# hbb1/2d-gaussian-splatting

Hardware: NVIDIA H100
Metric: fwd+bwd Msplats/sec at 1M surfels/1080p (higher is better)
Workload: dtype f32

## Files before the change

### 2d-gaussian-splatting_b200/csrc/api.cu

```cuda
#include <cstdarg>
#include <cstdio>
#include <cstring>
#include <cstdlib>
#include <algorithm>

#include "../../include/surfel_rasterizer.h"
#include "common.cuh"
#include "kernels.h"

using namespace surfel;

static thread_local char g_err[512] = "";

void surfel_set_error(const char* fmt, ...) {
    va_list ap;
    va_start(ap, fmt);
    vsnprintf(g_err, sizeof(g_err), fmt, ap);
    va_end(ap);
}

namespace {

struct Variants { int sort_radix; };
Variants& variants() {
    static Variants v = [] {
        auto is = [](const char* name, const char* val) { const char* e = getenv(name); return e && !strcmp(e, val) ? 1 : 0; };
        return Variants{is("SURFEL_SORT", "radix")};
    }();
    return v;
}

struct Frame { int W, H, gx, gy, row0, row1, tiles; };

bool frame_of(const surfel_settings_t* s, Frame& f) {
    if (!s) { surfel_set_error("settings is NULL"); return false; }
    f.W = s->image_width; f.H = s->image_height;
    if (f.W <= 0 || f.H <= 0) { surfel_set_error("bad image size %dx%d", f.W, f.H); return false; }
    f.gx = (f.W + kBlockX - 1) / kBlockX; f.gy = (f.H + kBlockY - 1) / kBlockY;
    f.tiles = f.gx * f.gy;
    f.row0 = s->tile_row_begin; f.row1 = s->tile_row_end;
    if (f.row0 == 0 && f.row1 == 0) f.row1 = f.gy;
    if (f.row0 < 0 || f.row1 > f.gy || f.row0 > f.row1) {
        surfel_set_error("bad tile row band [%d,%d) for %d tile rows", f.row0, f.row1, f.gy);
        return false;
    }
    return true;
}

int tile_key_bits(int tiles) {
    int b = 0;
    unsigned n = (unsigned)tiles;
    while (n) { b++; n >>= 1; }
    return 32 + b;
}

BinningLayout binning_layout(size_t R, int tiles) {
    BinningLayout L;
    size_t r = R > 0 ? R : 1, o = 0;
    L.keys_a = o;    o = align_up(o + r * 8, 256);
    L.keys_b = o;    o = align_up(o + r * 8, 256);
    L.vals_a = o;    o = align_up(o + r * 4, 256);
    L.vals_b = o;    o = align_up(o + r * 4, 256);
    L.ranges = o;    o = align_up(o + (size_t)tiles * 8, 256);
    L.sort_temp = o; o = align_up(o + std::max(radix_sort_temp_bytes(r), bucket_temp_bytes(tiles)), 256);
    L.total = o;
    return L;
}

struct BinView { uint64_t *k_unsorted, *k_sorted; uint32_t *v_unsorted, *v_sorted; uint64_t *k_a, *k_b; uint32_t *v_a, *v_b; uint2* ranges; void* temp; };

BinView bin_view(void* ws, size_t R, const Frame& f) {
    BinningLayout L = binning_layout(R, f.tiles);
    char* c = (char*)ws;
    BinView v;
    v.k_a = (uint64_t*)(c + L.keys_a); v.k_b = (uint64_t*)(c + L.keys_b);
    v.v_a = (uint32_t*)(c + L.vals_a); v.v_b = (uint32_t*)(c + L.vals_b);
    const bool in_b = radix_sort_passes(tile_key_bits(f.tiles)) & 1;
    v.k_unsorted = v.k_a; v.v_unsorted = v.v_a;
    v.k_sorted = in_b ? v.k_b : v.k_a; v.v_sorted = in_b ? v.v_b : v.v_a;
    v.ranges = (uint2*)(c + L.ranges);
    v.temp = c + L.sort_temp;
    return v;
}

uint32_t* mapped_alias(uint32_t* host) {
    if (!host) return nullptr;
    cudaPointerAttributes a;
    if (cudaPointerGetAttributes(&a, host) == cudaSuccess && a.type == cudaMemoryTypeHost && a.devicePointer)
        return (uint32_t*)a.devicePointer;
    (void)cudaGetLastError();
    return nullptr;
}

}

extern "C" {

int surfel_abi_version(void) { return SURFEL_ABI_VERSION; }

int surfel_set_variant(const char* name, const char* value) {
    if (!name || !value) { surfel_set_error("surfel_set_variant: NULL argument"); return 1; }
    Variants& v = variants();
    if (!strcmp(name, "sort")) {
        if (!strcmp(value, "bucket")) v.sort_radix = 0; else if (!strcmp(value, "radix")) v.sort_radix = 1; else goto bad;
    } else goto bad;
    return 0;
bad:
    surfel_set_error("surfel_set_variant: unknown variant %s=%s", name, value);
    return 1;
}
const char* surfel_last_error(void) { return g_err; }

int surfel_accepts_capacity(void) { return variants().sort_radix ? 0 : 1; }

size_t surfel_geom_bytes(int P) { return geom_layout(P).total; }
size_t surfel_image_bytes(int W, int H) { return image_layout(W, H).total; }
size_t surfel_binning_bytes(size_t R, int W, int H) {
    const int tiles = ((W + kBlockX - 1) / kBlockX) * ((H + kBlockY - 1) / kBlockY);
    return binning_layout(R, tiles).total;
}

int surfel_geom_offsets(int P, size_t* out) {
    GeomLayout L = geom_layout(P);
    out[0] = L.rec; out[1] = L.tiles_touched; out[2] = L.offsets; out[3] = L.clamped; out[4] = L.counters;
    out[5] = L.tmat;
    return 0;
}
int surfel_binning_offsets(size_t R, int W, int H, size_t* out) {
    const int tiles = ((W + kBlockX - 1) / kBlockX) * ((H + kBlockY - 1) / kBlockY);
    BinningLayout L = binning_layout(R, tiles);
    const bool in_b = radix_sort_passes(tile_key_bits(tiles)) & 1;
    out[0] = L.keys_a; out[1] = L.vals_a;
    out[2] = in_b ? L.keys_b : L.keys_a; out[3] = in_b ? L.vals_b : L.vals_a;
    out[4] = L.ranges;
    return 0;
}
int surfel_image_offsets(int W, int H, size_t* out) {
    ImageLayout L = image_layout(W, H);
    out[0] = L.accum; out[1] = L.n_contrib;
    return 0;
}

int surfel_forward_preprocess(const surfel_settings_t* s, int P, int M, const float* means3D,
                              const float* opacities, const float* scales, const float* rotations,
                              const float* transMat_precomp, const float* shs,
                              const float* colors_precomp, int32_t* radii, void* geom_ws, void* image_ws,
                              uint32_t* num_rendered_host, void* stream) {
    Frame f;
    if (!frame_of(s, f)) return 1;
    cudaStream_t st = (cudaStream_t)stream;
    if (P < 0) { surfel_set_error("P < 0"); return 1; }
    if (P > 0 && (!means3D || !opacities || !radii || !geom_ws)) { surfel_set_error("NULL required pointer"); return 1; }
    if (P > 0 && !transMat_precomp && (!scales || !rotations)) { surfel_set_error("need scales+rotations or transMat_precomp"); return 1; }
    if (P > 0 && !colors_precomp && !shs) { surfel_set_error("need shs or colors_precomp"); return 1; }
    if (!colors_precomp && (s->sh_degree < 0 || s->sh_degree > 3 || (s->sh_degree + 1) * (s->sh_degree + 1) > M)) {
        surfel_set_error("sh_degree %d unsupported for M=%d coefficients (max degree 3)", s->sh_degree, M);
        return 1;
    }
    GeomLayout L = geom_layout(P);
    char* g = (char*)geom_ws;
    if (P == 0) {
        if (num_rendered_host) *num_rendered_host = 0;
        return 0;
    }
    PreFwdParams p;
    p.P = P; p.D = s->sh_degree; p.M = M; p.W = f.W; p.H = f.H; p.gx = f.gx; p.gy = f.gy;
    p.row0 = f.row0; p.row1 = f.row1; p.prefiltered = s->prefiltered; p.scale_modifier = s->scale_modifier;
    p.means3D = means3D; p.scales = scales; p.rotations = rotations; p.opacities = opacities;
    p.shs = shs; p.transMat_precomp = transMat_precomp; p.colors_precomp = colors_precomp;
    p.viewmatrix = s->viewmatrix; p.projmatrix = s->projmatrix; p.campos = s->campos;
    p.radii = radii; p.rec = (float4*)(g + L.rec); p.tmat = (float4*)(g + L.tmat); p.tiles_touched = (uint32_t*)(g + L.tiles_touched);
    p.offsets = (uint32_t*)(g + L.offsets); p.clamped = (uint8_t*)(g + L.clamped);
    p.scan_status = (unsigned long long*)(g + L.scan_status); p.counters = (uint32_t*)(g + L.counters);
    p.tile_count = image_ws ? (uint32_t*)((char*)image_ws + image_layout(f.W, f.H).tile_count) : nullptr;
    p.num_rendered_mapped = mapped_alias(num_rendered_host);
    if (launch_preprocess_fwd(p, st)) return 1;
    if (num_rendered_host && !p.num_rendered_mapped)
        SURFEL_CUDA_OK(cudaMemcpyAsync(num_rendered_host, p.counters + 1, 4, cudaMemcpyDeviceToHost, st));
    return 0;
}

int surfel_bin_duplicate(const surfel_settings_t* s, int P, uint32_t R, const void* geom_ws,
                         const int32_t* radii, void* binning_ws, void* stream) {
    Frame f;
    if (!frame_of(s, f)) return 1;
    if (R == 0 || P == 0) return 0;
    GeomLayout L = geom_layout(P);
    const char* g = (const char*)geom_ws;
    BinView v = bin_view(binning_ws, R, f);
    return launch_duplicate_with_keys(P, f.gx, f.gy, f.row0, f.row1, (const float4*)(g + L.tmat), radii,
                                      (const uint32_t*)(g + L.offsets), v.k_unsorted, v.v_unsorted,
                                      (cudaStream_t)stream);
}

int surfel_bin_sort(const surfel_settings_t* s, uint32_t R, void* binning_ws, void* stream) {
    Frame f;
    if (!frame_of(s, f)) return 1;
    BinView v = bin_view(binning_ws, R, f);
    if (launch_radix_sort_pairs(v.k_a, v.v_a, v.k_b, v.v_b, R, tile_key_bits(f.tiles), v.temp,
                                (cudaStream_t)stream)) return 1;
    return launch_identify_tile_ranges(R, f.tiles, v.k_sorted, v.ranges, (cudaStream_t)stream);
}

int surfel_render_forward(const surfel_settings_t* s, uint32_t R, const void* geom_ws,
                          const void* binning_ws, void* image_ws, float* out_color,
                          float* out_others, void* stream) {
    Frame f;
    if (!frame_of(s, f)) return 1;
    BinView v = bin_view(const_cast<void*>(binning_ws), R, f);
    ImageLayout I = image_layout(f.W, f.H);
    RenderParams p;
    memset(&p, 0, sizeof(p));
    p.W = f.W; p.H = f.H; p.gx = f.gx; p.gy = f.gy; p.row0 = f.row0; p.row1 = f.row1;
    p.ranges = v.ranges; p.point_list = v.v_sorted;
    p.rec = (const float4*)((const char*)geom_ws + 0);
    p.bg = s->bg;
    p.out_color = out_color; p.out_others = out_others;
    p.out_plane = s->out_plane_stride > 0 ? (size_t)s->out_plane_stride : (size_t)f.W * f.H;
    if (p.out_plane < (size_t)f.W * f.H) { surfel_set_error("out_plane_stride smaller than the image"); return 1; }
    p.rep_count = s->out_replica_count;
    if (p.rep_count < 0 || p.rep_count > SURFEL_MAX_OUT_REPLICAS) { surfel_set_error("out_replica_count out of range"); return 1; }
    if (p.rep_count > 0 && out_others != out_color + 3 * p.out_plane) {
        surfel_set_error("out_replica_base needs out_others == out_color + 3 * out_plane_stride (one 10-plane frame)");
        return 1;
    }
    for (int r = 0; r < SURFEL_MAX_OUT_REPLICAS; r++) {
        p.rep_base[r] = r < p.rep_count ? (unsigned long long)s->out_replica_base[r] : 0ull;
        if (r < p.rep_count && (p.rep_base[r] == 0 || (p.rep_base[r] & 3ull))) { surfel_set_error("out_replica_base: null or misaligned address"); return 1; }
    }
    p.accum = (float*)((char*)image_ws + I.accum); p.n_contrib = (uint32_t*)((char*)image_ws + I.n_contrib);
    return launch_render_fwd(p, (cudaStream_t)stream);
}

int surfel_bin_bucket(const surfel_settings_t* s, int P, uint32_t R, const void* geom_ws,
                      const int32_t* radii, void* binning_ws, const void* image_ws_with_counts,
                      int write_keys, void* stream) {
    Frame f;
    if (!frame_of(s, f)) return 1;
    GeomLayout L = geom_layout(P);
    const char* g = (const char*)geom_ws;
    BinView v = bin_view(binning_ws, R, f);
    unsigned long long* pairs = (unsigned long long*)(v.k_sorted == v.k_a ? v.k_b : v.k_a);
    return launch_bucket_binning(P, R, f.gx, f.gy, f.row0, f.row1, (const float4*)(g + L.tmat), radii,
                                 (const uint32_t*)(g + L.offsets), pairs, v.v_sorted,
                                 write_keys ? (unsigned long long*)v.k_sorted : nullptr, v.ranges, v.temp,
                                 image_ws_with_counts ? (const uint32_t*)((const char*)image_ws_with_counts +
                                                                          image_layout(f.W, f.H).tile_count) : nullptr,
                                 (cudaStream_t)stream);
}

int surfel_forward_render(const surfel_settings_t* s, int P, uint32_t R, const int32_t* radii,
                          const void* geom_ws, void* binning_ws, void* image_ws, int tile_counts_ready,
                          float* out_color, float* out_others, void* stream) {
    const bool use_radix = variants().sort_radix != 0;
    if (!use_radix) {
        if (surfel_bin_bucket(s, P, R, geom_ws, radii, binning_ws, tile_counts_ready ? image_ws : nullptr, 0, stream)) return 1;
        return surfel_render_forward(s, R, geom_ws, binning_ws, image_ws, out_color, out_others, stream);
    }
    if (surfel_bin_duplicate(s, P, R, geom_ws, radii, binning_ws, stream)) return 1;
    if (surfel_bin_sort(s, R, binning_ws, stream)) return 1;
    return surfel_render_forward(s, R, geom_ws, binning_ws, image_ws, out_color, out_others, stream);
}

int surfel_backward(const surfel_settings_t* s, int P, int M, uint32_t R, const float* means3D,
                    const float* scales, const float* rotations, const float* transMat_precomp,
                    const float* shs, int has_colors_precomp, const int32_t* radii,
                    const void* geom_ws, const void* binning_ws, const void* image_ws,
                    const float* dL_dout_color, const float* dL_dout_others, float* grad_scratch,
                    float* dL_dmeans2D, float* dL_dcolors, float* dL_dopacity, float* dL_dmeans3D,
                    float* dL_dtransMat, float* dL_dsh, float* dL_dscales, float* dL_drotations,
                    int lowpass_depth_quirk, void* stream) {
    Frame f;
    if (!frame_of(s, f)) return 1;
    if (P <= 0) return 0;
    cudaStream_t st = (cudaStream_t)stream;
    if (!grad_scratch || !dL_dmeans2D || !dL_dopacity || !dL_dmeans3D) { surfel_set_error("NULL required gradient buffer"); return 1; }
    GeomLayout L = geom_layout(P);
    const char* g = (const char*)geom_ws;
    SURFEL_CUDA_OK(cudaMemsetAsync(grad_scratch, 0, (size_t)P * kGradFloats * 4, st));
    if (R > 0) {
        BinView v = bin_view(const_cast<void*>(binning_ws), R, f);
        ImageLayout I = image_layout(f.W, f.H);
        RenderParams p;
        memset(&p, 0, sizeof(p));
        p.W = f.W; p.H = f.H; p.gx = f.gx; p.gy = f.gy; p.row0 = f.row0; p.row1 = f.row1;
        p.ranges = v.ranges; p.point_list = v.v_sorted; p.rec = (const float4*)(g + L.rec); p.bg = s->bg;
        p.accum = (float*)((char*)image_ws + I.accum); p.n_contrib = (uint32_t*)((char*)image_ws + I.n_contrib);
        p.dL_dpix = dL_dout_color; p.dL_dothers = dL_dout_others; p.grad_rec = grad_scratch;
        p.grad_plane = s->grad_plane_stride > 0 ? (size_t)s->grad_plane_stride : (size_t)f.W * f.H;
        if (p.grad_plane < (size_t)f.W * f.H) { surfel_set_error("grad_plane_stride smaller than the image"); return 1; }
        p.lowpass_quirk = lowpass_depth_quirk;
        if (launch_render_bwd(p, st)) return 1;
    }
    PreBwdParams q;
    memset(&q, 0, sizeof(q));
    q.P = P; q.D = s->sh_degree; q.M = M; q.W = f.W; q.H = f.H; q.scale_modifier = s->scale_modifier;
    q.means3D = means3D; q.scales = scales; q.rotations = rotations; q.shs = shs;
    q.transMat_precomp = transMat_precomp; q.has_colors_precomp = has_colors_precomp;
    q.viewmatrix = s->viewmatrix; q.projmatrix = s->projmatrix; q.campos = s->campos;
    q.radii = radii; q.tmat = (const float4*)(g + L.tmat); q.clamped = (const uint8_t*)(g + L.clamped);
    q.grad_rec = grad_scratch;
    q.dL_dmeans2D = dL_dmeans2D; q.dL_dcolors = dL_dcolors; q.dL_dopacity = dL_dopacity;
    q.dL_dmeans3D = dL_dmeans3D; q.dL_dtransMat = dL_dtransMat; q.dL_dsh = dL_dsh;
    q.dL_dscales = dL_dscales; q.dL_drots = dL_drotations;
    q.defer_sh = (s->sh_grad_deferred && shs != nullptr && !has_colors_precomp) ? 1 : 0;
    if (q.defer_sh && !dL_dcolors) { surfel_set_error("sh_grad_deferred needs dL_dcolors"); return 1; }
    return launch_preprocess_bwd(q, st);
}

int surfel_sh_grad_expand(int P, int M, int sh_degree, const float* means3D, const float* campos,
                          const float* dL_dcolors, float* dL_dsh, void* stream) {
    if (P <= 0 || M <= 0) return 0;
    if (!means3D || !campos || !dL_dcolors || !dL_dsh) { surfel_set_error("surfel_sh_grad_expand: NULL argument"); return 1; }
    if (sh_degree < 0 || sh_degree > 3 || (sh_degree + 1) * (sh_degree + 1) > M) { surfel_set_error("surfel_sh_grad_expand: degree / M mismatch"); return 1; }
    return launch_sh_grad_expand(P, M, sh_degree, means3D, campos, dL_dcolors, dL_dsh, (cudaStream_t)stream);
}

int surfel_mark_visible(int P, const float* means3D, const float* viewmatrix,
                        const float* projmatrix, uint8_t* present, void* stream) {
    (void)projmatrix;
    return launch_mark_visible(P, means3D, viewmatrix, present, (cudaStream_t)stream);
}

size_t surfel_sort_temp_bytes(size_t n) { return radix_sort_temp_bytes(n); }
int surfel_grad_scratch_floats(void) { return kGradFloats; }

int surfel_sort_pairs(uint64_t* keys_a, uint32_t* vals_a, uint64_t* keys_b, uint32_t* vals_b,
                      size_t n, int end_bit, void* temp, int* result_in_b, void* stream) {
    if (result_in_b) *result_in_b = radix_sort_passes(end_bit) & 1;
    return launch_radix_sort_pairs(keys_a, vals_a, keys_b, vals_b, n, end_bit, temp, (cudaStream_t)stream);
}

}
```

### 2d-gaussian-splatting_b200/csrc/common.cuh

```cuda
#pragma once
#include <cuda_runtime.h>
#include <stdint.h>

namespace surfel {

constexpr int kBlockX = 16;
constexpr int kBlockY = 16;
constexpr int kTilePixels = kBlockX * kBlockY;
constexpr float kNear = 0.2f;
constexpr float kFar = 100.0f;
constexpr float kFilterSize = 0.707106f;
constexpr float kFilterInvSquare = 2.0f;
constexpr float kCutoff = 3.0f;
constexpr float kAlphaMax = 0.99f;
constexpr float kAlphaMin = 1.0f / 255.0f;
constexpr float kTMin = 0.0001f;

constexpr int kChDepth = 0, kChAlpha = 1, kChNormal = 2, kChMidDepth = 5, kChDistortion = 6;

constexpr int kRecQuads = 8;
constexpr int kRecBytes = kRecQuads * 16;
constexpr int kRecQuadsFwd = 5;
constexpr int kRecQuadsBwd = 6;

constexpr int kTmQuads = 3;

constexpr int kGradFloats = 24;
constexpr int kGradUsed = 22;

struct GeomLayout {
    size_t rec, tmat, tiles_touched, offsets, clamped, scan_status, counters, total;
};
struct ImageLayout {
    size_t accum, n_contrib, tile_count, total;
};
struct BinningLayout {
    size_t keys_a, keys_b, vals_a, vals_b, ranges, sort_temp, total;
};

__host__ __device__ inline size_t align_up(size_t x, size_t a) { return (x + a - 1) / a * a; }

constexpr int kPreBlock = 128;

inline GeomLayout geom_layout(int P) {
    GeomLayout L;
    size_t o = 0;
    size_t p = (size_t)(P > 0 ? P : 1);
    L.rec = o;            o = align_up(o + p * kRecBytes, 256);
    L.tmat = o;           o = align_up(o + p * kTmQuads * 16, 256);
    L.tiles_touched = o;  o = align_up(o + p * 4, 256);
    L.offsets = o;        o = align_up(o + p * 4, 256);
    L.clamped = o;        o = align_up(o + p, 256);
    L.scan_status = o;    o = align_up(o + ((p + kPreBlock - 1) / kPreBlock + 1) * 8, 256);
    L.counters = o;       o = align_up(o + 64, 256);
    L.total = o;
    return L;
}
inline ImageLayout image_layout(int W, int H) {
    ImageLayout L;
    size_t n = (size_t)W * (size_t)H;
    size_t o = 0;
    L.accum = o;      o = align_up(o + n * 3 * 4, 256);
    L.n_contrib = o;  o = align_up(o + n * 2 * 4, 256);
    const size_t tiles = (size_t)((W + kBlockX - 1) / kBlockX) * (size_t)((H + kBlockY - 1) / kBlockY);
    L.tile_count = o; o = align_up(o + tiles * 4, 256);
    L.total = o;
    return L;
}

__device__ __forceinline__ int f2i_sat(float x) { return __float2int_rz(x); }

__device__ __forceinline__ void get_rect(float cx, float cy, int radius, int gx, int gy, int row0,
                                         int row1, int& x0, int& y0, int& x1, int& y1) {
    const float r = (float)radius;
    x0 = min(gx, max(0, f2i_sat((cx - r) / (float)kBlockX)));
    y0 = min(gy, max(0, f2i_sat((cy - r) / (float)kBlockY)));
    x1 = min(gx, max(0, f2i_sat(((cx + r) + (float)(kBlockX - 1)) / (float)kBlockX)));
    y1 = min(gy, max(0, f2i_sat(((cy + r) + (float)(kBlockY - 1)) / (float)kBlockY)));
    y0 = min(row1, max(row0, y0));
    y1 = min(row1, max(row0, y1));
}

__device__ __forceinline__ float4 ld_nc_f4(const float4* p) {
    float4 r;
    asm volatile("ld.global.nc.L1::no_allocate.v4.f32 {%0,%1,%2,%3}, [%4];"
                 : "=f"(r.x), "=f"(r.y), "=f"(r.z), "=f"(r.w) : "l"(p));
    return r;
}

}

void surfel_set_error(const char* fmt, ...);

constexpr int kMaxDevices = 64;
inline int current_device_slot() {
    int dev = -1;
    if (cudaGetDevice(&dev) != cudaSuccess || dev < 0 || dev >= kMaxDevices) return -1;
    return dev;
}
inline int current_device_sm_count() {
    static int cached[kMaxDevices] = {};
    const int slot = current_device_slot();
    if (slot >= 0 && cached[slot] > 0) return cached[slot];
    int dev = 0, n = 0;
    if (cudaGetDevice(&dev) != cudaSuccess || cudaDeviceGetAttribute(&n, cudaDevAttrMultiProcessorCount, dev) != cudaSuccess || n <= 0)
        n = 132;
    if (slot >= 0) cached[slot] = n;
    return n;
}
#define SURFEL_CUDA_OK(expr)                                                              \
    do {                                                                                  \
        cudaError_t _e = (expr);                                                          \
        if (_e != cudaSuccess) {                                                          \
            surfel_set_error("%s failed: %s (%s:%d)", #expr, cudaGetErrorString(_e),      \
                             __FILE__, __LINE__);                                         \
            return 1;                                                                     \
        }                                                                                 \
    } while (0)
```

### 2d-gaussian-splatting_b200/csrc/kernels.h

```cpp
#pragma once
#include <cuda_runtime.h>
#include <stdint.h>
#include <stddef.h>

namespace surfel {

struct PreFwdParams {
    int P, D, M, W, H, gx, gy, row0, row1, prefiltered;
    float scale_modifier;
    const float* means3D; const float* scales; const float* rotations; const float* opacities;
    const float* shs; const float* transMat_precomp; const float* colors_precomp;
    const float* viewmatrix; const float* projmatrix; const float* campos;
    int* radii; float4* rec; float4* tmat; uint32_t* tiles_touched; uint32_t* offsets; uint8_t* clamped;
    unsigned long long* scan_status; uint32_t* counters;
    uint32_t* tile_count;
    uint32_t* num_rendered_mapped;
};

struct PreBwdParams {
    int P, D, M, W, H;
    float scale_modifier;
    const float* means3D; const float* scales; const float* rotations; const float* shs;
    const float* transMat_precomp; int has_colors_precomp;
    const float* viewmatrix; const float* projmatrix; const float* campos;
    const int* radii; const float4* tmat; const uint8_t* clamped;
    const float* grad_rec;
    float* dL_dmeans2D;
    float* dL_dcolors;
    float* dL_dopacity;
    float* dL_dmeans3D;
    float* dL_dtransMat;
    float* dL_dsh;
    float* dL_dscales;
    float* dL_drots;
    int defer_sh;
};

struct RenderParams {
    int W, H, gx, gy, row0, row1;
    const uint2* ranges; const uint32_t* point_list; const float4* rec;
    const float* bg;
    float* out_color; float* out_others; float* accum; uint32_t* n_contrib;
    const float* dL_dpix; const float* dL_dothers; float* grad_rec; int lowpass_quirk;
    size_t out_plane, grad_plane;
    int rep_count; unsigned long long rep_base[8];
};

int launch_preprocess_fwd(const PreFwdParams& p, cudaStream_t stream);
int launch_mark_visible(int P, const float* means3D, const float* viewmatrix, uint8_t* present,
                        cudaStream_t stream);
int launch_preprocess_bwd(const PreBwdParams& p, cudaStream_t stream);
int launch_sh_grad_expand(int P, int M, int D, const float* means3D, const float* campos,
                          const float* dL_dcolors, float* dL_dsh, cudaStream_t stream);

int launch_duplicate_with_keys(int P, int gx, int gy, int row0, int row1, const float4* tmat,
                               const int* radii, const uint32_t* offsets, uint64_t* keys,
                               uint32_t* vals, cudaStream_t stream);
int launch_identify_tile_ranges(size_t R, int tiles, const uint64_t* keys_sorted, uint2* ranges,
                                cudaStream_t stream);

size_t radix_sort_temp_bytes(size_t n);
int radix_sort_passes(int end_bit);
int launch_radix_sort_pairs(uint64_t* keys_a, uint32_t* vals_a, uint64_t* keys_b,
                            uint32_t* vals_b, size_t n, int end_bit, void* temp,
                            cudaStream_t stream);

size_t bucket_temp_bytes(int tiles);
int launch_bucket_binning(int P, size_t R, int gx, int gy, int row0, int row1, const float4* tmat,
                          const int* radii, const uint32_t* offsets, unsigned long long* pairs,
                          uint32_t* point_list, unsigned long long* keys_sorted, uint2* ranges,
                          void* temp, const uint32_t* tile_count_ready, cudaStream_t stream);

int launch_render_fwd(const RenderParams& p, cudaStream_t stream);
int launch_render_bwd(const RenderParams& p, cudaStream_t stream);

}
```

### 2d-gaussian-splatting_b200/csrc/render_bwd.cu

```cuda
#include "render_common.cuh"
#include "kernels.h"
#include "profile.h"

namespace surfel {

#ifndef SURFEL_BWD_BLOCKS
#define SURFEL_BWD_BLOCKS 4
#endif
#ifndef SURFEL_BWD_BATCH
#define SURFEL_BWD_BATCH 256
#endif
constexpr int kBatchB = SURFEL_BWD_BATCH;
constexpr int kGroupsB = kBatchB / 32;
constexpr int kPanelRow = 24;
constexpr int kPanelBytes = 8 * 32 * kPanelRow * 4;
constexpr int kRecBytesB = kRecQuadsFwd * kBatchB * 16;
constexpr int kBwdSmemBytes = kRecBytesB + kBatchB * 4 + kPanelBytes + 8 * kGroupsB * 4 + 32;

__device__ __forceinline__ float column_sum(uint32_t a, int cnt) {
    float acc = 0.0f, acc2 = 0.0f;
    int r = cnt;
#pragma unroll 1
    for (; r >= 4; r -= 4, a += 4 * kPanelRow * 4) {
        const float x0 = lds32(a), x1 = lds32(a + kPanelRow * 4), x2 = lds32(a + 2 * kPanelRow * 4), x3 = lds32(a + 3 * kPanelRow * 4);
        acc += x0 + x1; acc2 += x2 + x3;
    }
#pragma unroll 1
    for (; r > 0; r--, a += kPanelRow * 4) acc += lds32(a);
    return acc + acc2;
}

__global__ void __launch_bounds__(256, SURFEL_BWD_BLOCKS) render_bwd_kernel(RenderParams p) {
    extern __shared__ __align__(16) unsigned char smem_raw[];
    float4* s_rec = reinterpret_cast<float4*>(smem_raw);
    uint32_t* s_id = reinterpret_cast<uint32_t*>(smem_raw + kRecBytesB);
    float* s_panel = reinterpret_cast<float*>(smem_raw + kRecBytesB + kBatchB * 4);
    uint32_t* s_mask = reinterpret_cast<uint32_t*>(smem_raw + kRecBytesB + kBatchB * 4 + kPanelBytes);
    uint32_t* s_max = s_mask + 8 * kGroupsB;

    const int tid = threadIdx.x, lane = tid & 31, warp = tid >> 5;
    const int tx = blockIdx.x, ty = blockIdx.y + p.row0;
    int lx, ly;
    warp_pixel(warp, lane, lx, ly);
    const int px = tx * kBlockX + lx, py = ty * kBlockY + ly;
    const bool inside = px < p.W && py < p.H;
    const float pxf = (float)px, pyf = (float)py;
    const float ox = (float)(tx * kBlockX), oy = (float)(ty * kBlockY);
    const uint2 range = p.ranges[ty * p.gx + tx];
    const size_t HW = (size_t)p.H * p.W;
    const size_t pix = (size_t)py * p.W + px;
    const uint32_t rec_base = smem_u32(s_rec);
    uint32_t panel_base = smem_u32(s_panel) + warp * (32 * kPanelRow * 4);
    const uint32_t id_base = smem_u32(s_id);
    const uint32_t mask_base = smem_u32(s_mask) + (uint32_t)warp * (kGroupsB * 4);
    unsigned lt_mask = (1u << lane) - 1u;

    float T_final = 0, final_D = 0, final_D2 = 0;
    uint32_t last_contributor = 0, median_contributor = 0;
    float dpix0 = 0, dpix1 = 0, dpix2 = 0, dN0 = 0, dN1 = 0, dN2 = 0;
    float dL_ddepth = 0, dL_daccum = 0, dL_dreg = 0, dL_dmedian = 0;
    if (inside) {
        T_final = p.accum[pix]; final_D = p.accum[HW + pix]; final_D2 = p.accum[2 * HW + pix];
        last_contributor = p.n_contrib[pix]; median_contributor = p.n_contrib[HW + pix];
        const size_t GP = p.grad_plane;
        dpix0 = p.dL_dpix[pix]; dpix1 = p.dL_dpix[GP + pix]; dpix2 = p.dL_dpix[2 * GP + pix];
        dL_ddepth = p.dL_dothers[kChDepth * GP + pix];
        dL_daccum = p.dL_dothers[kChAlpha * GP + pix];
        dN0 = p.dL_dothers[(kChNormal + 0) * GP + pix];
        dN1 = p.dL_dothers[(kChNormal + 1) * GP + pix];
        dN2 = p.dL_dothers[(kChNormal + 2) * GP + pix];
        dL_dmedian = p.dL_dothers[kChMidDepth * GP + pix];
        dL_dreg = p.dL_dothers[kChDistortion * GP + pix];
    }
    const float Ar = (1.0f - T_final) * dL_dreg, Ar2 = Ar + Ar, nD1r2 = -2.0f * final_D * dL_dreg, D2r = final_D2 * dL_dreg;
    const uint32_t median_index = median_contributor - 1u;
    const bool quirk = p.lowpass_quirk != 0;

    uint32_t warp_max = last_contributor;
#pragma unroll
    for (int o = 16; o > 0; o >>= 1) warp_max = max(warp_max, __shfl_xor_sync(0xffffffffu, warp_max, o));
    if (lane == 0) s_max[warp] = warp_max;
    __syncthreads();
    uint32_t cta_max = 0;
#pragma unroll
    for (int w = 0; w < 8; w++) cta_max = max(cta_max, s_max[w]);

    float T = T_final;
    float S = T_final * ((__ldg(p.bg + 0) * dpix0 + __ldg(p.bg + 1) * dpix1) + __ldg(p.bg + 2) * dpix2);
    constexpr float kMScale = kFar / (kFar - kNear);
    constexpr float kDmScale = (kFar * kNear) / (kFar - kNear);

    for (int end = (int)cta_max; end > 0; end -= kBatchB) {
        const int n = min(kBatchB, end);
        const int start = end - n;
        if (end != (int)cta_max) __syncthreads();
#pragma unroll
        for (int k = 0; k < (kBatchB + 255) / 256; k++) {
            const int slot = k * 256 + tid;
            if (k * 256 + (warp << 5) >= n) break;
            uint32_t m8 = 0;
            if (slot < n) {
                const uint32_t id = __ldg(p.point_list + range.x + start + slot);
                const float4* r = p.rec + (size_t)id * kRecQuads;
                const float4 bb = __ldg(r + 6), dg = __ldg(r + 7);
#ifdef SURFEL_STAGE_LDG
#pragma unroll
                for (int q = 0; q < kRecQuadsFwd; q++) s_rec[q * kBatchB + slot] = __ldg(r + q);
#else
#pragma unroll
                for (int q = 0; q < kRecQuadsFwd; q++) cp_async16(rec_base + (uint32_t)(q * kBatchB + slot) * 16u, r + q);
#endif
                s_id[slot] = id;
                m8 = classify_footprints(bb, dg, ox, oy);
            }
            uint32_t keep = 0;
#pragma unroll
            for (int w = 0; w < 8; w++) {
                const uint32_t b = __ballot_sync(0xffffffffu, (m8 >> w) & 1u);
                if (lane == w) keep = b;
            }
            if (lane < 8) s_mask[lane * kGroupsB + k * 8 + warp] = keep;
        }
        cp_async_wait_all();
        __syncthreads();
        if ((int)warp_max <= start) continue;

        const int top = min(n, (int)warp_max - start);
        for (int g = (top - 1) >> 5; g >= 0; g--) {
            unsigned m = lds32u(mask_base + (uint32_t)g * 4u) & low_mask((uint32_t)(top - (g << 5)));
            uint32_t gb = rec_base + (uint32_t)(g << 5) * 16u, idb = id_base + (uint32_t)(g << 5) * 4u;
            asm volatile("" : "+r"(gb), "+r"(idb), "+r"(panel_base), "+r"(lt_mask));
            const int own = (int)last_contributor - (start + (g << 5));
            const int med = (int)median_index - (start + (g << 5));
            while (m) {
                const uint32_t j = high_bit(m);
                m &= low_mask(j);
                const uint32_t ra = gb + j * 16u;
                const float4 q0 = lds128(ra), q1 = lds128(ra + kBatchB * 16), q2 = lds128(ra + 2 * kBatchB * 16);
                PairEval e;
                const bool active = eval_pair(pxf, pyf, q0, q1, q2, e) && (int)j < own;
                const unsigned am = __ballot_sync(0xffffffffu, active);
                if (am == 0u) continue;

                if (active) {
                    const float4 q3 = lds128(ra + 3 * kBatchB * 16), q4 = lds128(ra + 4 * kBatchB * 16);
                    const bool use3d = e.rho3d <= e.rho2d;
                    const float depth = use3d ? q4.w * e.inv_pz : q3.w;
                    const uint32_t ro = panel_base + (uint32_t)__popc(am & lt_mask) * (kPanelRow * 4);
                    if (q2.w < 0.0f && depth < kNear) {
                        const float4 z4 = make_float4(0.f, 0.f, 0.f, 0.f);
                        sts128(ro, z4); sts128(ro + 16, z4); sts128(ro + 32, z4); sts128(ro + 48, z4); sts128(ro + 64, z4);
                        sts64(ro + 80, 0.f, 0.f);
                    } else {
                        float ax = 0, ay = 0, az = 0, zd = 0, zx = 0, zy = 0, zz = 0, m2x = 0, m2y = 0;
                        const float G = e.G, alpha = e.alpha;
                        const float inv1ma = fast_rcp(1.0f - alpha);
                        T = T * inv1ma;
                        const float w = alpha * T;
                        const float inv_d = fast_rcp(depth);
                        const float m_d = fmaf(inv_d, -kMScale * kNear, kMScale);
                        const float dmd_dd = kDmScale * inv_d * inv_d;
                        float v = fmaf(m_d, fmaf(m_d, Ar, nD1r2), D2r) + dL_daccum;
                        v = fmaf(q4.x, dpix0, v); v = fmaf(q4.y, dpix1, v); v = fmaf(q4.z, dpix2, v);
                        v = fmaf(depth, dL_ddepth, v);
                        v = fmaf(q3.x, dN0, v); v = fmaf(q3.y, dN1, v); v = fmaf(q3.z, dN2, v);
                        const float dL_dalpha = fmaf(T, v, -(S * inv1ma));
                        S = fmaf(w, v, S);
                        float dL_dz = ((int)j == med) ? dL_dmedian : 0.0f;
                        dL_dz = fmaf(w * dmd_dd, fmaf(m_d, Ar2, nD1r2), dL_dz);
                        const float dL_dG = fabsf(q2.w) * dL_dalpha;
                        dL_dz = fmaf(w, dL_ddepth, dL_dz);
                        const float dop = G * dL_dalpha;
                        if (use3d) {
                            const float t = -G * dL_dG * e.inv_pz;
                            ax = t * e.sx; ay = t * e.sy;
                            zd = dL_dz * e.inv_pz;
                            az = -fmaf(ax, e.sx, fmaf(ay, e.sy, zd * depth));
                        } else {
                            const float gg = G * kFilterInvSquare * dL_dG;
                            m2x = gg * e.dx; m2y = gg * e.dy;
                            zz = dL_dz;
                            if (quirk) { zx = e.sx * dL_dz; zy = e.sy * dL_dz; }
                        }
                        sts128(ro, make_float4(ax, ay, az, e.dx * ax));
                        sts128(ro + 16, make_float4(e.dx * ay, e.dx * az, e.dy * ax, e.dy * ay));
                        sts128(ro + 32, make_float4(e.dy * az, zd, zx, zy));
                        sts128(ro + 48, make_float4(zz, m2x, m2y, dop));
                        sts128(ro + 64, make_float4(w * dN0, w * dN1, w * dN2, w * dpix0));
                        sts64(ro + 80, w * dpix1, w * dpix2);
                    }
                }
                const uint32_t id = lds32u(idb + j * 4u);
                __syncwarp();
                {
                    const float acc = column_sum(panel_base + (uint32_t)min(__popc(lt_mask), kPanelRow - 1) * 4u, __popc(am));
                    if (lane < kGradUsed && acc != 0.0f) {
                        atomicAdd(p.grad_rec + (size_t)id * kGradFloats + lane, acc);
                    }
                }
                __syncwarp();
            }
        }
    }
}

int launch_render_bwd(const RenderParams& p, cudaStream_t stream) {
    const int rows = p.row1 - p.row0;
    if (rows <= 0 || p.gx <= 0) return 0;
    static bool attr_set[kMaxDevices] = {};
    const int slot = current_device_slot();
    if (slot < 0 || !attr_set[slot]) {
        SURFEL_CUDA_OK(cudaFuncSetAttribute(render_bwd_kernel, cudaFuncAttributeMaxDynamicSharedMemorySize, kBwdSmemBytes));
        if (slot >= 0) attr_set[slot] = true;
    }
    dim3 grid(p.gx, rows);
    LaunchScope scope(kStRenderBwd, stream);
    render_bwd_kernel<<<grid, 256, kBwdSmemBytes, stream>>>(p);
    SURFEL_CUDA_OK(cudaGetLastError());
    return 0;
}

}
```

### 2d-gaussian-splatting_b200/csrc/render_fwd_tile.inc

```
    float4* s_rec = reinterpret_cast<float4*>(smem_raw);
    uint32_t* s_mask = reinterpret_cast<uint32_t*>(smem_raw + kRecQuadsFwd * kBatch * 16);

    const int tid = threadIdx.x, lane = tid & 31, warp = tid >> 5;
    int lx, ly;
    warp_pixel(warp, lane, lx, ly);
    const int px = tx * kBlockX + lx, py = ty * kBlockY + ly;
    const bool inside = px < p.W && py < p.H;
    const float pxf = (float)px, pyf = (float)py;
    const float ox = (float)(tx * kBlockX), oy = (float)(ty * kBlockY);

    const uint2 range = p.ranges[ty * p.gx + tx];
    const int total = (int)(range.y - range.x);
    const uint32_t rec_base = smem_u32(s_rec);
    const uint32_t mask_base = smem_u32(s_mask) + (uint32_t)warp * (kGroups * 4);
    constexpr float kMScale = kFar / (kFar - kNear);

    float T = 1.0f, C0 = 0, C1 = 0, C2 = 0, N0 = 0, N1 = 0, N2 = 0, D = 0, M1 = 0, M2 = 0, dist = 0;
    float median_depth = 0;
    uint32_t last_contributor = inside ? 0u : 0x80000000u;
    uint32_t median_contributor = 0xFFFFFFFFu;
    bool warp_done = __all_sync(0xffffffffu, !inside);

    for (int base = 0; base < total; base += kBatch) {
        if (base > 0 && !__syncthreads_or(!warp_done)) break;

        const int n = min(kBatch, total - base);
#pragma unroll
        for (int k = 0; k < (kBatch + 255) / 256; k++) {
            const int slot = k * 256 + tid;
            if (k * 256 + (warp << 5) >= n) break;
            uint32_t m8 = 0;
            if (slot < n) {
                const uint32_t id = __ldg(p.point_list + range.x + base + slot);
                const float4* r = p.rec + (size_t)id * kRecQuads;
                const float4 bb = __ldg(r + 6), dg = __ldg(r + 7);
#ifdef SURFEL_STAGE_LDG
#pragma unroll
                for (int q = 0; q < kRecQuadsFwd; q++) s_rec[q * kBatch + slot] = __ldg(r + q);
#else
#pragma unroll
                for (int q = 0; q < kRecQuadsFwd; q++) cp_async16(rec_base + (uint32_t)(q * kBatch + slot) * 16u, r + q);
#endif
                m8 = classify_footprints(bb, dg, ox, oy);
            }
            uint32_t keep = 0;
#pragma unroll
            for (int w = 0; w < 8; w++) {
                const uint32_t b = __ballot_sync(0xffffffffu, (m8 >> w) & 1u);
                if (lane == w) keep = b;
            }
            if (lane < 8) s_mask[lane * kGroups + k * 8 + warp] = __brev(keep);
        }
        cp_async_wait_all();
        __syncthreads();

        if (!warp_done) {
            const int ngroups = (n + 31) >> 5;
            for (int g = 0; g < ngroups; g++) {
                unsigned m = lds32u(mask_base + (uint32_t)g * 4u);
                if ((int)last_contributor >= 0) {
                    const uint32_t g31 = rec_base + (uint32_t)(g * 32 + 31) * 16u;
                    const uint32_t k32 = (uint32_t)(base + g * 32 + 32);
                    while (m) {
                        const uint32_t hb = high_bit(m);
                        m &= low_mask(hb);
                        const uint32_t ra = g31 - hb * 16u;
                        const float4 q0 = lds128(ra), q1 = lds128(ra + kBatch * 16), q2 = lds128(ra + 2 * kBatch * 16);
                        PairEval e;
                        if (!eval_pair(pxf, pyf, q0, q1, q2, e)) continue;
                        const float4 q3 = lds128(ra + 3 * kBatch * 16), q4 = lds128(ra + 4 * kBatch * 16);
                        const float depth = (e.rho3d <= e.rho2d) ? q4.w * e.inv_pz : q3.w;
                        if (q2.w < 0.0f && depth < kNear) continue;
                        const float test_T = T * (1.0f - e.alpha);
                        if (test_T < kTMin) { last_contributor |= 0x80000000u; break; }
                        const uint32_t contributor = k32 - hb;
                        const float w = e.alpha * T;
                        const float A = 1.0f - T;
                        const float mm = fmaf(fast_rcp(depth), -kMScale * kNear, kMScale);
                        dist = fmaf(fmaf(mm, fmaf(mm, A, -(M1 + M1)), M2), w, dist);
                        D += depth * w;
                        M1 += mm * w;
                        M2 += mm * mm * w;
                        if (T > 0.5f) { median_depth = depth; median_contributor = contributor; }
                        N0 += q3.x * w; N1 += q3.y * w; N2 += q3.z * w;
                        C0 += q4.x * w; C1 += q4.y * w; C2 += q4.z * w;
                        T = test_T;
                        last_contributor = contributor;
                    }
                }
                if (__all_sync(0xffffffffu, (int)last_contributor < 0)) { warp_done = true; break; }
            }
        }
    }
```

Measured before the change: 471.8.

## Record per-warp blended masks in forward and reuse them to skip dead splats in backward

The forward render now writes, for every 32-splat group and warp, a bitmask of the splats that were actually blended into a per-tile live buffer in the binning workspace. The backward pass reads these masks instead of re-running footprint classification. It only stages rec data for splats live in some warp, which cuts global loads, cp.async traffic and mask-walk work. The cost is extra global stores in the forward, more workspace, and a dependency on the forward having been run with the same binning buffers. The loop start is also rounded to a multiple of 32.

```diff
diff --git a/2d-gaussian-splatting_b200/csrc/api.cu b/2d-gaussian-splatting_b200/csrc/api.cu
--- a/2d-gaussian-splatting_b200/csrc/api.cu
+++ b/2d-gaussian-splatting_b200/csrc/api.cu
@@ -63,11 +63,12 @@
     L.vals_b = o;    o = align_up(o + r * 4, 256);
     L.ranges = o;    o = align_up(o + (size_t)tiles * 8, 256);
     L.sort_temp = o; o = align_up(o + std::max(radix_sort_temp_bytes(r), bucket_temp_bytes(tiles)), 256);
+    L.live = o;      o = align_up(o + ((r >> 5) + (size_t)tiles + 1) * 8 * 4, 256);
     L.total = o;
     return L;
 }
 
-struct BinView { uint64_t *k_unsorted, *k_sorted; uint32_t *v_unsorted, *v_sorted; uint64_t *k_a, *k_b; uint32_t *v_a, *v_b; uint2* ranges; void* temp; };
+struct BinView { uint64_t *k_unsorted, *k_sorted; uint32_t *v_unsorted, *v_sorted; uint64_t *k_a, *k_b; uint32_t *v_a, *v_b; uint2* ranges; void* temp; uint32_t* live; };
 
 BinView bin_view(void* ws, size_t R, const Frame& f) {
     BinningLayout L = binning_layout(R, f.tiles);
@@ -80,6 +81,7 @@
     v.k_sorted = in_b ? v.k_b : v.k_a; v.v_sorted = in_b ? v.v_b : v.v_a;
     v.ranges = (uint2*)(c + L.ranges);
     v.temp = c + L.sort_temp;
+    v.live = (uint32_t*)(c + L.live);
     return v;
 }
 
@@ -212,7 +214,7 @@
     RenderParams p;
     memset(&p, 0, sizeof(p));
     p.W = f.W; p.H = f.H; p.gx = f.gx; p.gy = f.gy; p.row0 = f.row0; p.row1 = f.row1;
-    p.ranges = v.ranges; p.point_list = v.v_sorted;
+    p.ranges = v.ranges; p.point_list = v.v_sorted; p.live = v.live;
     p.rec = (const float4*)((const char*)geom_ws + 0);
     p.bg = s->bg;
     p.out_color = out_color; p.out_others = out_others;
@@ -284,7 +286,7 @@
         RenderParams p;
         memset(&p, 0, sizeof(p));
         p.W = f.W; p.H = f.H; p.gx = f.gx; p.gy = f.gy; p.row0 = f.row0; p.row1 = f.row1;
-        p.ranges = v.ranges; p.point_list = v.v_sorted; p.rec = (const float4*)(g + L.rec); p.bg = s->bg;
+        p.ranges = v.ranges; p.point_list = v.v_sorted; p.live = v.live; p.rec = (const float4*)(g + L.rec); p.bg = s->bg;
         p.accum = (float*)((char*)image_ws + I.accum); p.n_contrib = (uint32_t*)((char*)image_ws + I.n_contrib);
         p.dL_dpix = dL_dout_color; p.dL_dothers = dL_dout_others; p.grad_rec = grad_scratch;
         p.grad_plane = s->grad_plane_stride > 0 ? (size_t)s->grad_plane_stride : (size_t)f.W * f.H;
diff --git a/2d-gaussian-splatting_b200/csrc/common.cuh b/2d-gaussian-splatting_b200/csrc/common.cuh
--- a/2d-gaussian-splatting_b200/csrc/common.cuh
+++ b/2d-gaussian-splatting_b200/csrc/common.cuh
@@ -35,7 +35,7 @@
     size_t accum, n_contrib, tile_count, total;
 };
 struct BinningLayout {
-    size_t keys_a, keys_b, vals_a, vals_b, ranges, sort_temp, total;
+    size_t keys_a, keys_b, vals_a, vals_b, ranges, sort_temp, live, total;
 };
 
 __host__ __device__ inline size_t align_up(size_t x, size_t a) { return (x + a - 1) / a * a; }
diff --git a/2d-gaussian-splatting_b200/csrc/kernels.h b/2d-gaussian-splatting_b200/csrc/kernels.h
--- a/2d-gaussian-splatting_b200/csrc/kernels.h
+++ b/2d-gaussian-splatting_b200/csrc/kernels.h
@@ -41,6 +41,7 @@
     const uint2* ranges; const uint32_t* point_list; const float4* rec;
     const float* bg;
     float* out_color; float* out_others; float* accum; uint32_t* n_contrib;
+    uint32_t* live;
     const float* dL_dpix; const float* dL_dothers; float* grad_rec; int lowpass_quirk;
     size_t out_plane, grad_plane;
     int rep_count; unsigned long long rep_base[8];
diff --git a/2d-gaussian-splatting_b200/csrc/render_bwd.cu b/2d-gaussian-splatting_b200/csrc/render_bwd.cu
--- a/2d-gaussian-splatting_b200/csrc/render_bwd.cu
+++ b/2d-gaussian-splatting_b200/csrc/render_bwd.cu
@@ -45,7 +45,6 @@
     const int px = tx * kBlockX + lx, py = ty * kBlockY + ly;
     const bool inside = px < p.W && py < p.H;
     const float pxf = (float)px, pyf = (float)py;
-    const float ox = (float)(tx * kBlockX), oy = (float)(ty * kBlockY);
     const uint2 range = p.ranges[ty * p.gx + tx];
     const size_t HW = (size_t)p.H * p.W;
     const size_t pix = (size_t)py * p.W + px;
@@ -84,25 +83,29 @@
     uint32_t cta_max = 0;
 #pragma unroll
     for (int w = 0; w < 8; w++) cta_max = max(cta_max, s_max[w]);
+    const uint32_t lane_max = lane < 8 ? s_max[lane] : 0u;
+    const uint32_t* live = p.live + 8 * ((size_t)(range.x >> 5) + (size_t)(ty * p.gx + tx)) + lane;
 
     float T = T_final;
     float S = T_final * ((__ldg(p.bg + 0) * dpix0 + __ldg(p.bg + 1) * dpix1) + __ldg(p.bg + 2) * dpix2);
     constexpr float kMScale = kFar / (kFar - kNear);
     constexpr float kDmScale = (kFar * kNear) / (kFar - kNear);
 
-    for (int end = (int)cta_max; end > 0; end -= kBatchB) {
+    const int list_end = ((int)cta_max + 31) & ~31;
+    for (int end = list_end; end > 0; end -= kBatchB) {
         const int n = min(kBatchB, end);
         const int start = end - n;
-        if (end != (int)cta_max) __syncthreads();
+        if (end != list_end) __syncthreads();
 #pragma unroll
         for (int k = 0; k < (kBatchB + 255) / 256; k++) {
             const int slot = k * 256 + tid;
             if (k * 256 + (warp << 5) >= n) break;
-            uint32_t m8 = 0;
-            if (slot < n) {
+            const int G = (start >> 5) + k * 8 + warp;
+            const uint32_t keep = (uint32_t)(G << 5) < lane_max ? __ldg(live + 8 * G) : 0u;
+            if (lane < 8) s_mask[lane * kGroupsB + k * 8 + warp] = keep;
+            if ((__reduce_or_sync(0xffffffffu, keep) >> lane) & 1u) {
                 const uint32_t id = __ldg(p.point_list + range.x + start + slot);
                 const float4* r = p.rec + (size_t)id * kRecQuads;
-                const float4 bb = __ldg(r + 6), dg = __ldg(r + 7);
 #ifdef SURFEL_STAGE_LDG
 #pragma unroll
                 for (int q = 0; q < kRecQuadsFwd; q++) s_rec[q * kBatchB + slot] = __ldg(r + q);
@@ -111,15 +114,7 @@
                 for (int q = 0; q < kRecQuadsFwd; q++) cp_async16(rec_base + (uint32_t)(q * kBatchB + slot) * 16u, r + q);
 #endif
                 s_id[slot] = id;
-                m8 = classify_footprints(bb, dg, ox, oy);
             }
-            uint32_t keep = 0;
-#pragma unroll
-            for (int w = 0; w < 8; w++) {
-                const uint32_t b = __ballot_sync(0xffffffffu, (m8 >> w) & 1u);
-                if (lane == w) keep = b;
-            }
-            if (lane < 8) s_mask[lane * kGroupsB + k * 8 + warp] = keep;
         }
         cp_async_wait_all();
         __syncthreads();
@@ -127,7 +122,7 @@
 
         const int top = min(n, (int)warp_max - start);
         for (int g = (top - 1) >> 5; g >= 0; g--) {
-            unsigned m = lds32u(mask_base + (uint32_t)g * 4u) & low_mask((uint32_t)(top - (g << 5)));
+            unsigned m = lds32u(mask_base + (uint32_t)g * 4u);
             uint32_t gb = rec_base + (uint32_t)(g << 5) * 16u, idb = id_base + (uint32_t)(g << 5) * 4u;
             asm volatile("" : "+r"(gb), "+r"(idb), "+r"(panel_base), "+r"(lt_mask));
             const int own = (int)last_contributor - (start + (g << 5));
diff --git a/2d-gaussian-splatting_b200/csrc/render_fwd_tile.inc b/2d-gaussian-splatting_b200/csrc/render_fwd_tile.inc
--- a/2d-gaussian-splatting_b200/csrc/render_fwd_tile.inc
+++ b/2d-gaussian-splatting_b200/csrc/render_fwd_tile.inc
@@ -13,6 +13,7 @@
     const int total = (int)(range.y - range.x);
     const uint32_t rec_base = smem_u32(s_rec);
     const uint32_t mask_base = smem_u32(s_mask) + (uint32_t)warp * (kGroups * 4);
+    const uint32_t live_word = 8u * ((range.x >> 5) + (uint32_t)(ty * p.gx + tx)) + (uint32_t)warp;
     constexpr float kMScale = kFar / (kFar - kNear);
 
     float T = 1.0f, C0 = 0, C1 = 0, C2 = 0, N0 = 0, N1 = 0, N2 = 0, D = 0, M1 = 0, M2 = 0, dist = 0;
@@ -58,6 +59,7 @@
             const int ngroups = (n + 31) >> 5;
             for (int g = 0; g < ngroups; g++) {
                 unsigned m = lds32u(mask_base + (uint32_t)g * 4u);
+                uint32_t blended = 0;
                 if ((int)last_contributor >= 0) {
                     const uint32_t g31 = rec_base + (uint32_t)(g * 32 + 31) * 16u;
                     const uint32_t k32 = (uint32_t)(base + g * 32 + 32);
@@ -86,8 +88,11 @@
                         C0 += q4.x * w; C1 += q4.y * w; C2 += q4.z * w;
                         T = test_T;
                         last_contributor = contributor;
+                        blended |= 0x80000000u >> hb;
                     }
                 }
+                const uint32_t wm = __reduce_or_sync(0xffffffffu, blended);
+                if (lane == 0) p.live[live_word + 8u * (uint32_t)((base >> 5) + g)] = wm;
                 if (__all_sync(0xffffffffu, (int)last_contributor < 0)) { warp_done = true; break; }
             }
         }
diff --git a/profiles/hit_census.py b/profiles/hit_census.py
--- /dev/null
+++ b/profiles/hit_census.py
@@ -0,0 +1,164 @@
+import os
+import sys
+import time
+
+import numpy as np
+
+ROOT = os.path.dirname(os.path.dirname(os.path.abspath(__file__)))
+sys.path[:0] = [ROOT, os.path.join(ROOT, "2d-gaussian-splatting_b200")]
+
+NEAR = 0.2
+ALPHA_MIN = 1.0 / 255.0
+
+
+def footprint_bounds(pre):
+    tm = pre["transMat"].astype(np.float64)
+    c = pre["xy"].astype(np.float64)
+    cx, cy = c[:, 0], c[:, 1]
+    opa = pre["normal_opacity"][:, 3].astype(np.float64)
+    P = tm.shape[0]
+    ext = np.empty((P, 8))
+    a255 = 255.0 * opa
+    with np.errstate(all="ignore"):
+        tau = 2.0 * np.log(np.maximum(a255, 1e-30)) + 0.01
+        r2 = np.sqrt(np.maximum(0.5 * tau, 0.0)) + 0.05
+        r2d = r2 * 1.41421366
+        ext[:] = np.stack([-r2, r2, -r2, r2, -r2d, r2d, -r2d, r2d], 1)
+        Tw = tm[:, 6:9]
+        tu = tm[:, 0:3] - cx[:, None] * Tw
+        tv = tm[:, 3:6] - cy[:, None] * Tw
+        wxy = Tw[:, 0] ** 2 + Tw[:, 1] ** 2
+        wz2 = Tw[:, 2] ** 2
+        bounded = (Tw[:, 2] > 0) & (wz2 > 1.05 * tau * wxy)
+        d = tau * wxy - wz2
+        f0, f2 = tau / d, -1.0 / d
+        for k, (nx, ny) in enumerate(((1.0, 0.0), (0.0, 1.0), (1.0, 1.0), (1.0, -1.0))):
+            a = nx * tu + ny * tv
+            ec = f0 * (a[:, 0] * Tw[:, 0] + a[:, 1] * Tw[:, 1]) + f2 * (a[:, 2] * Tw[:, 2])
+            ee = f0 * (a[:, 0] ** 2 + a[:, 1] ** 2) + f2 * a[:, 2] ** 2
+            eh = np.sqrt(np.maximum(0.0, ec * ec - ee))
+            mg = 0.05 + 1e-4 * (np.abs(ec) + eh)
+            bounded &= np.isfinite(ec) & np.isfinite(eh)
+            lo, hi = np.minimum(ext[:, 2 * k], ec - eh - mg), np.maximum(ext[:, 2 * k + 1], ec + eh + mg)
+            ext[:, 2 * k] = np.where(bounded, lo, ext[:, 2 * k])
+            ext[:, 2 * k + 1] = np.where(bounded, hi, ext[:, 2 * k + 1])
+    ext[~bounded] = np.array([-3e38, 3e38] * 4)
+    ext[a255 < 0.999] = np.array([3e38, -3e38] * 4)
+    cu, cv = cx + cy, cx - cy
+    bb = np.stack([cx + ext[:, 0], cy + ext[:, 2], cx + ext[:, 1], cy + ext[:, 3]], 1)
+    dg = np.stack([cu + ext[:, 4], cu + ext[:, 5], cv + ext[:, 6], cv + ext[:, 7]], 1)
+    tau_n = 2.0 * np.log(np.maximum(a255, 1.0)) + 0.01
+    flagged = Tw[:, 2] - np.sqrt(tau_n * wxy) < NEAR * 1.001
+    return bb, dg, flagged
+
+
+def classify(bb, dg, ox, oy):
+    x0, x1, y0, y1 = bb[:, 0] - ox, bb[:, 2] - ox, bb[:, 1] - oy, bb[:, 3] - oy
+    u0, u1, v0, v1 = dg[:, 0] - (ox + oy), dg[:, 1] - (ox + oy), dg[:, 2] - (ox - oy), dg[:, 3] - (ox - oy)
+    out = np.zeros((bb.shape[0], 8), bool)
+    for w in range(8):
+        fx0, fy0 = float((w & 1) << 3), float((w >> 1) << 2)
+        fx1, fy1 = fx0 + 7.0, fy0 + 3.0
+        out[:, w] = ((x0 <= fx1) & (x1 >= fx0) & (y0 <= fy1) & (y1 >= fy0) & (u0 <= fx1 + fy1) & (u1 >= fx0 + fy0)
+                     & (v0 <= fx1 - fy0) & (v1 >= fx0 - fy1))
+    return out
+
+
+def warp_lane_pixels():
+    w, l = np.meshgrid(np.arange(8), np.arange(32), indexing="ij")
+    return ((w & 1) << 3) + (l & 7), ((w >> 1) << 2) + (l >> 3)
+
+
+def tile_masks(pre, ids, n_contrib, W, H, tx, ty):
+    lx, ly = warp_lane_pixels()
+    px, py = tx * 16 + lx, ty * 16 + ly
+    inside = (px < W) & (py < H)
+    nc = np.where(inside, n_contrib[np.minimum(py, H - 1), np.minimum(px, W - 1)], 0).astype(np.int64)
+    pxf, pyf = px.astype(np.float64)[None], py.astype(np.float64)[None]
+    T = pre["transMat"][ids].astype(np.float64)
+    Tu, Tv, Tw = (T[:, None, None, 3 * i:3 * i + 3] for i in range(3))
+    k = pxf[..., None] * Tw - Tu
+    l = pyf[..., None] * Tw - Tv
+    p = np.cross(k, l)
+    with np.errstate(all="ignore"):
+        sx, sy = p[..., 0] / p[..., 2], p[..., 1] / p[..., 2]
+        rho3d = sx * sx + sy * sy
+        c = pre["xy"][ids].astype(np.float64)
+        rho2d = 2.0 * ((c[:, 0, None, None] - pxf) ** 2 + (c[:, 1, None, None] - pyf) ** 2)
+        alpha = np.minimum(0.99, pre["normal_opacity"][ids, 3].astype(np.float64)[:, None, None]
+                           * np.exp(-0.5 * np.minimum(rho3d, rho2d)))
+        depth = np.where(rho3d <= rho2d, sx * Tw[..., 0] + sy * Tw[..., 1] + Tw[..., 2], Tw[..., 2])
+    slot = np.arange(len(ids))[:, None, None]
+    active = (alpha >= ALPHA_MIN) & (p[..., 2] != 0) & (slot < nc[None])
+    return active, depth < NEAR, nc.max(axis=1)
+
+
+def census(pre, binned, n_contrib, W, H, tile_stride=1):
+    bb, dg, flagged = footprint_bounds(pre)
+    gx = (W + 15) // 16
+    c = dict(tiles=0, slots_total=0, slots_staged=0, slots_live=0, hits=0, hits_dead=0, hits_live=0,
+             hits_blended=0, lanes_live=0, pairs_blended=0, blended_unclassified=0)
+    for tile in range(0, binned["ranges"].shape[0], tile_stride):
+        a, b = (int(v) for v in binned["ranges"][tile])
+        if b <= a:
+            continue
+        tx, ty = tile % gx, tile // gx
+        ids = binned["vals_sorted"][a:b]
+        active, near, warp_max = tile_masks(pre, ids, n_contrib, W, H, tx, ty)
+        blended = active & ~(near & flagged[ids][:, None, None])
+        cls = classify(bb[ids], dg[ids], float(tx * 16), float(ty * 16))
+        slot = np.arange(len(ids))[:, None]
+        walked = cls & (slot < warp_max[None, :])
+        am = active.sum(axis=2)
+        live = blended.any(axis=2)
+        c["tiles"] += 1
+        c["slots_total"] += len(ids)
+        c["slots_staged"] += int(warp_max.max())
+        c["slots_live"] += int(live.any(axis=1).sum())
+        c["hits"] += int(walked.sum())
+        c["hits_dead"] += int((walked & (am == 0)).sum())
+        c["hits_live"] += int((walked & (am > 0)).sum())
+        c["hits_blended"] += int(live.sum())
+        c["lanes_live"] += int(am[walked & (am > 0)].sum())
+        c["pairs_blended"] += int(blended.sum())
+        c["blended_unclassified"] += int((live & ~walked).sum())
+    return c
+
+
+def report(c):
+    h = max(c["hits"], 1)
+    lines = [
+        f"tiles                       {c['tiles']}",
+        f"warp-hits walked            {c['hits']}",
+        f"  dead (am == 0)            {c['hits_dead']}  ({100.0 * c['hits_dead'] / h:.1f} %)",
+        f"  live (am != 0)            {c['hits_live']}  (mean popc(am) {c['lanes_live'] / max(c['hits_live'], 1):.2f})",
+        f"  blended by the forward    {c['hits_blended']}",
+        f"slots in the tile lists     {c['slots_total']}",
+        f"slots staged today          {c['slots_staged']}",
+        f"slots live in some warp     {c['slots_live']}  ({100.0 * (1 - c['slots_live'] / max(c['slots_staged'], 1)):.1f} % of staged are not needed)",
+    ]
+    return "\n".join(lines)
+
+
+def main():
+    import surfel_scenes as S
+    from oracle import surfel_oracle as O
+    name = sys.argv[1] if len(sys.argv) > 1 else "headline"
+    stride = int(sys.argv[2]) if len(sys.argv) > 2 else 1
+    scene, cam = S.named(name)
+    scene = S.to_numpy(scene)
+    W, H = cam["W"], cam["H"]
+    t0 = time.time()
+    pre = O.preprocess_fwd(scene["means3D"], scene["scales"], scene["rotations"], scene["opacities"], scene["shs"],
+                           cam["viewmatrix"], cam["projmatrix"], cam["campos"], W, H, 3, 1.0)
+    binned = O.bin_sort(pre, W, H)
+    img = O.render_fwd(pre, binned, np.zeros(3, np.float32), W, H)
+    print(f"# hit census, {name}: P={len(scene['means3D'])} {W}x{H} R={binned['R']} tile stride {stride}"
+          f" (oracle {time.time() - t0:.0f} s)")
+    c = census(pre, binned, img["n_contrib"][0], W, H, stride)
+    print(report(c))
+    print(f"# {time.time() - t0:.0f} s")
+
+
+if __name__ == "__main__":
+    main()
```

After: 489.3, median of 6. 1.04x the previous value.
